# AnimatePortrait/AnimatePortrait

Measured on AMD Instinct MI355X. Metric: generator frames/sec @256x256 bs=16, higher is better.
Workload: dtype f32 (fp32 tensors; wide convs multiply fp32-class on the bf16 pipe: operands as bf16 head + tail, 3 products of 16-bit significands per multiply, ~2^-17 relative per product, fp32 accumulate); 1 GPU; Module2 generator resnet_9blocks_rcatland32_full_ifw fwd-only, ngf=64, bs=16/GPU, 256x256, fp32 (BASELINE configs[1]); global_batch=16, parallelism=dp1 (frame batches sharded, no collective), weights=random init N(0,0.02), seed 1234

## Files before the change

animateportrait_amd/csrc/conv_bf16x3.h:

```cpp
#pragma once
#include <type_traits>
#include <utility>

#include "conv_igemm.h"

namespace apamd {

typedef __bf16 bf16x8 __attribute__((ext_vector_type(8)));

template <int S_, int K_, int WCO_, int MT_, int WPX_, int NT_, int NTAP_ = 0, int ROW_ = 0, int PARTS_ = 2, int S2D3_ = 0,
          int OB16_ = 0>
struct Bf3Cfg {
    static constexpr int OB16 = OB16_;
    static_assert(!OB16_ || (K_ == 3 && S_ == 1 && PARTS_ == 1 && !ROW_), "bf16 output: the plain-bf16 3x3 stride-1 tiles");
    static constexpr int CI = 16, S = S_, K = K_, WCO = WCO_, MT = MT_, WPX = WPX_, NT = NT_, ROW = ROW_, PARTS = PARTS_;
    static constexpr int S2D3 = S2D3_;
    static_assert(!S2D3_ || (K_ == 0 && NTAP_ == 4), "compile-time s2d tap sets: the 4-tap run-time-tap family");
    static_assert(PARTS == 1 || PARTS == 2, "head only, or head + tail");
    static constexpr int TMAX = K > 0 ? (ROW ? K : K * K) : NTAP_;
    static_assert(TMAX >= 1, "K == 0 needs a tap count");
    static constexpr int EXT = K > 0 ? K - 1 : 1;
    static constexpr int EXTY = (K > 0 && ROW) ? 0 : EXT;
    static constexpr int TH = WPX * NT;
    static constexpr int CO_TILE = WCO * MT * 32;
    static constexpr int IH = (TH - 1) * S + EXTY + 1;
    static constexpr int IW = 31 * S + EXT + 1;
    static constexpr int PLANE = IH * IW;
    static constexpr int XP = (2 * PLANE + 63) / 64 * 64;
    static constexpr int X_SLOTS = PARTS * XP;
    static int w_slots(int ntaps) { return PARTS * ntaps * 2 * CO_TILE; }
    static constexpr int NIT = XP / 256 + (XP % 256 ? 1 : 0);
    static constexpr int W_BYTES_MAX = PARTS * TMAX * 2 * CO_TILE * 16;
    static constexpr int NPATCH = (NT % 2 == 0 && (8 * 32 * 36 + WPX * CO_TILE * 2) * 4 <= PARTS * XP * 16 + W_BYTES_MAX) ? 2 : 1;
    static constexpr int EPI_FLOATS = 4 * NPATCH * 32 * 36 + WPX * CO_TILE * 2;
    static_assert(WCO * WPX == 4, "4 waves per workgroup");
    static_assert(CO_TILE % 16 == 0, "weight image must be whole wave-wide LDS-DMA pieces");
    static_assert(IH < 128 && IW < 256, "piece geometry is packed into 15 bits");
    static constexpr int WG_PER_CU = (PARTS == 1 || 2 * (X_SLOTS + PARTS * TMAX * 2 * CO_TILE) * 16 + 1024 <= 80 * 1024) ? 2 : 1;
    static int wfloats(int ntaps) { return 2 * ntaps * 2 * CO_TILE * 4; }
    static size_t lds_bytes(int ntaps) {
        const size_t stage = (size_t)(X_SLOTS + w_slots(ntaps)) * 16, epi = (size_t)EPI_FLOATS * 4;
        return 2 * stage + (epi > stage ? (epi - stage + 15) / 16 * 16 : 0);
    }
};

__device__ __forceinline__ void split_bf16(float v, __bf16& hi, __bf16& lo) {
    hi = (__bf16)v;
    lo = (__bf16)(v - (float)hi);
}

struct Bf3Tile {
    int n, cot, ty, tx;
};

__device__ __forceinline__ void glds16_sv(const void* sbase, unsigned voff, unsigned lds_addr) {
    asm volatile("s_mov_b32 m0, %2\n\ts_nop 0\n\tglobal_load_lds_dwordx4 %0, %1" ::"v"(voff), "s"(sbase), "s"(lds_addr)
                 : "memory", "m0");
}
template <int IMM>
__device__ __forceinline__ void glds16_si(const void* sbase, unsigned voff, unsigned lds_base) {
    asm volatile("s_add_u32 m0, %2, %3\n\ts_nop 0\n\tglobal_load_lds_dwordx4 %0, %1" ::"v"(voff), "s"(sbase), "s"(lds_base), "n"(IMM)
                 : "memory", "m0", "scc");
}
__device__ __forceinline__ void dma_wait_all() { asm volatile("s_waitcnt vmcnt(0)" ::: "memory"); }

template <class F, int... J>
__device__ __forceinline__ void static_for_impl(F&& f, std::integer_sequence<int, J...>) {
    (f(std::integral_constant<int, J>{}), ...);
}
template <int N, class F>
__device__ __forceinline__ void static_for(F&& f) {
    static_for_impl(static_cast<F&&>(f), std::make_integer_sequence<int, N>{});
}

template <class C>
__global__ __launch_bounds__(256, C::WG_PER_CU) void conv_bf16x3(const ConvKParams p) {
    constexpr int S = C::S, K = C::K, TMAX = C::TMAX, MT = C::MT, NT = C::NT, WCO = C::WCO;
// ... 78 lines not shown
        if (p.nseg > 1 && chunk >= p.seg[1].chunk_begin) s = 1;
        if (p.nseg > 2 && chunk >= p.seg[2].chunk_begin) s = 2;
        return s;
    };

    int pgeo[NIT];
#pragma unroll
    for (int k = 0; k < NIT; ++k) {
        const int it = tid + k * 256;
        const int kg = it >= PLANE ? 1 : 0;
        const int pix = it - kg * PLANE;
        const int ly = pix / IW;
        int lx = pix - ly * IW;
        if constexpr (S == 2) lx = lx < IWE ? 2 * lx : 2 * (lx - IWE) + 1;
        pgeo[k] = it < 2 * PLANE ? ((kg << 15) | (ly << 8) | lx) : -1;
    }
    auto locate = [&](int logical, Bf3Tile& t, int (&goff)[NIT]) __attribute__((always_inline)) {
        t.cot = logical % p.co_tiles;
        int t_ = logical / p.co_tiles;
        t.tx = t_ % p.tiles_x;
        t_ /= p.tiles_x;
        t.ty = t_ % p.tiles_y;
        t.n = t_ / p.tiles_y;
        int dy0 = p.dy0, dx0 = p.dx0;
        if (p.nphase > 1) {
            const int ph = t.cot / p.co_tiles_phase;
            dy0 = p.ph_dy0[ph];
            dx0 = p.ph_dx0[ph];
        }
        const int iy0 = t.ty * C::TH * S + dy0, ix0 = t.tx * 32 * S + dx0;
#pragma unroll
        for (int k = 0; k < NIT; ++k) {
            int gy = iy0 + ((pgeo[k] >> 8) & 127), gx = ix0 + (pgeo[k] & 255);
            bool ok = pgeo[k] >= 0;
            if (p.pad_mode == 1) {
                gy = reflect_clamp(gy, H);
                gx = reflect_clamp(gx, W);
            } else {
                ok = ok && gy >= 0 && gy < H && gx >= 0 && gx < W;
            }
            goff[k] = (ok ? ((pgeo[k] >> 15) & 1) * (HW + 1) + gy * W + gx : HW) * 16;
        }
    };
    struct DmaCtx {
        const unsigned char* xh;
        const unsigned char* xl;
        const unsigned char* wsrc;
        unsigned xdst, wdst;
        unsigned wmask;
    };
    constexpr int NWP = (W_SLOTS / 64 + 3) / 4, NPIECE = PARTS * NIT + NWP;
    unsigned woff[NWP];
#pragma unroll
    for (int j = 0; j < NWP; ++j) woff[j] = ((j * 4 + wave) * 64 + lane) * 16;
    auto dma_setup = [&](int n, int cot, int chunk_, int buf) __attribute__((always_inline)) {
        const int chunk = chunk_ < nreal ? chunk_ : nreal - 1;
        const int s = seg_of(chunk);
        const int cg0 = (chunk - p.seg[s].chunk_begin) * 2;
        const int CG = p.seg[s].C >> 3;
        const unsigned char* xs = reinterpret_cast<const unsigned char*>(p.seg[s].data);
        const unsigned char* xh = xs + ((long long)(n * 2 + 0) * CG + cg0) * (HW + 1) * 16;
        const unsigned char* xl = xs + ((long long)(n * 2 + 1) * CG + cg0) * (HW + 1) * 16;
        unsigned xdst = lds0 + (buf * STAGE + W_SLOTS + wave * 64) * 16;
        const unsigned char* wsrc = reinterpret_cast<const unsigned char*>(p.wp + ((long long)cot * nchunks + chunk_) * p.wfloats);
        unsigned wdst = lds0 + (buf * STAGE + wave * 64) * 16;
        unsigned wmask = 0xFu;
        if constexpr (C::S2D3) wmask = p.s2d_mask[chunk_ / p.s2d_div < 3 ? chunk_ / p.s2d_div : 3];
        asm volatile("" : "+s"(xh), "+s"(xl), "+s"(wsrc), "+s"(xdst), "+s"(wdst));
        return DmaCtx{xh, xl, wsrc, xdst, wdst, wmask};
    };
    auto dma_piece = [&](const DmaCtx& d, const int (&goff)[NIT], const int (&alt)[NIT], bool use_alt, auto jt) __attribute__((always_inline)) {
        constexpr int j = decltype(jt)::value;
        if constexpr (j < PARTS * NIT) {
            constexpr int part = j / NIT, k = j % NIT;
            constexpr bool whole = k * 256 + 3 * 64 < XP;
            if (whole || k * 256 + wave * 64 < XP)
                glds16_si<(part * XP + k * 256) * 16>(part ? d.xl : d.xh, (unsigned)(use_alt ? alt[k] : goff[k]), d.xdst);
        } else {
            constexpr int jj = j - PARTS * NIT;
            constexpr bool whole = jj * 4 + 3 < W_SLOTS / 64;
            bool want = whole || jj * 4 + wave < W_SLOTS / 64;
            if constexpr (C::S2D3) want = want && ((d.wmask >> (((jj * 4 + wave) % (T * 2 * CO_TILE / 64)) / (2 * CO_TILE / 64))) & 1u);
            if (want) glds16_si<jj * 4096>(d.wsrc, woff[jj], d.wdst);
        }
    };
    auto issue = [&](const Bf3Tile& t, const int (&goff)[NIT], int chunk_, int buf) __attribute__((always_inline)) {
        const DmaCtx d = dma_setup(t.n, t.cot, chunk_, buf);
        static_for<NPIECE>([&](auto jt) __attribute__((always_inline)) { dma_piece(d, goff, goff, false, jt); });
    };

    const int a_slot = half * CO_TILE + wco * MT * 32 + l32;
    const int b_slot = half * PLANE + (wpx * NT) * S * IW + (S == 2 ? l32 : l32 * S);

    f32x16 acc[MT][NT];
    bf16x8 ah[2][MT], al[2][MT], bh[2][NT], bl[2][NT];
    constexpr bool WIN = (K == 4 || (K == 3 && NT > 1)) && !C::ROW && S == 1;
    constexpr int WR = WIN ? NT + K - 1 : 1;
    bf16x8 wh[2][WR], wl[2][WR];
    auto fetch_a = [&](int stage_buf, int t, int buf) __attribute__((always_inline)) {
        const uint4* Wc = wbuf + stage_buf * STAGE + a_slot;
#pragma unroll
        for (int m = 0; m < MT; ++m) {
            ah[buf][m] = *reinterpret_cast<const bf16x8*>(Wc + ((0 * T + t) * 2) * CO_TILE + m * 32);
            if constexpr (PARTS == 2) al[buf][m] = *reinterpret_cast<const bf16x8*>(Wc + ((1 * T + t) * 2) * CO_TILE + m * 32);
        }
    };
    auto fetch_brow = [&](int stage_buf, int kx, int j, int wb) __attribute__((always_inline)) {
        const uint4* Xc = xbuf + stage_buf * STAGE + b_slot + j * IW + kx;
        wh[wb][j] = *reinterpret_cast<const bf16x8*>(Xc);
        if constexpr (PARTS == 2) wl[wb][j] = *reinterpret_cast<const bf16x8*>(Xc + XP);
    };
    auto fetch = [&](int stage_buf, int t, int buf) __attribute__((always_inline)) {
        const uint4* Wc = wbuf + stage_buf * STAGE + a_slot;
        const uint4* Xc = xbuf + stage_buf * STAGE + b_slot;
        int toff;
        if constexpr (K > 0) toff = C::ROW ? t : (t / K) * IW + (S == 2 ? ((t % K) & 1) * IWE + ((t % K) >> 1) : (t % K));
        else toff = (int)((p.tap_bits >> (2 * t)) & 1u) * IW + (int)((p.tap_bits >> (2 * t + 1)) & 1u);
// ... 192 lines not shown
            }
            for (; c < 2 * cpp; c += 2) {
                stage(P0{}, std::integral_constant<unsigned, 0x5u>{}, c);
                stage(P1{}, std::integral_constant<unsigned, 0x5u>{}, c + 1);
            }
            for (; c < 3 * cpp; c += 2) {
                stage(P0{}, std::integral_constant<unsigned, 0x3u>{}, c);
                stage(P1{}, std::integral_constant<unsigned, 0x3u>{}, c + 1);
            }
            for (; c < nchunks; c += 2) {
                stage(P0{}, std::integral_constant<unsigned, 0x1u>{}, c);
                stage(P1{}, std::integral_constant<unsigned, 0x1u>{}, c + 1);
            }
        } else {
            for (int c = 0; c < nchunks; c += 2) {
                stage(P0{}, std::integral_constant<unsigned, 0u>{}, c);
                stage(P1{}, std::integral_constant<unsigned, 0u>{}, c + 1);
            }
        }
        AP_STAMP(3, 0);
        constexpr int pl = 1;

        auto epilogue = [&](auto atag) __attribute__((always_inline)) {
            constexpr int ACT = decltype(atag)::value;
            auto actf = [&](float v) { return ACT >= 0 ? apply_act(v, ACT) : apply_act(v, p.act); };
            constexpr int TS = 36;
            float* const epi = reinterpret_cast<float*>(smem + pl * STAGE);
            constexpr int NP = C::NPATCH;
            float* const patch0 = epi + wave * (NP * 32 * TS);
            float* const sred = epi + 4 * NP * 32 * TS;
            const int n = cur.n;
            int cot = cur.cot, oy_off = p.oy_off, ox_off = p.ox_off, stat_off = p.stat_tile_off;
            if (p.nphase > 1) {
                const int ph = cot / p.co_tiles_phase;
                cot -= ph * p.co_tiles_phase;
                oy_off = p.ph_oy[ph];
                ox_off = p.ph_ox[ph];
                stat_off = p.ph_stat[ph];
            }
            const int oy0 = cur.ty * C::TH, ox0 = cur.tx * 32;
            const int co_base = cot * CO_TILE + wco * MT * 32;
            const bool want_stats = p.stats != nullptr;
            const bool vec_ok = ((p.o_rstride | (int)p.o_cstride | (int)p.o_nstride) & 3) == 0 && p.osx == 1 && ox_off == 0 &&
                                (reinterpret_cast<uintptr_t>(p.y) & 15) == 0;
            const bool full = vec_ok && ox0 + 32 <= p.OW;
            const int prow = lane >> 3, pcol = (lane & 7) * 4;
            const int oxv = ox0 + pcol;
            bool octet = false;
            if constexpr (C::K == 0 || C::ROW || (C::K == 3 && C::S == 1 && C::PARTS == 2 && !C::OB16)) {
                octet = p.o_octet != 0;
                if (octet) {
                    const int ox = ox0 + l32;
                    const long long ohw = (long long)p.OH * p.OW;
                    const bool allv = !(C::WG_PER_CU == 2 && (C::K == 0 || (C::ROW && C::MT == 2))) &&
                                      __builtin_amdgcn_readfirstlane((int)(p.bias == nullptr && ACT == 0 && co_base + MT * 32 <= p.Cout &&
                                                                           oy0 + C::TH <= p.OH && ox0 + 32 <= p.OW)) != 0;
#pragma unroll
                    for (int m = 0; m < MT; ++m) {
                        float s16[16], q16[16];
#pragma unroll
                        for (int r = 0; r < 16; ++r) { s16[r] = 0.f; q16[r] = 0.f; }
                        if (allv) {
#pragma unroll
                            for (int g = 0; g < 4; ++g) {
                                const int co = co_base + m * 32 + g * 8 + 4 * half;
                                float* const ob = p.y + (long long)n * p.o_nstride + (long long)(co >> 3) * ohw * 8 + (co & 7) +
                                                  ((long long)(oy0 + wpx * NT) * p.OW + ox) * 8;
#pragma unroll
                                for (int q = 0; q < NT; ++q) {
                                    float vv[4];
#pragma unroll
                                    for (int j = 0; j < 4; ++j) {
                                        vv[j] = acc[m][q][g * 4 + j];
                                        s16[g * 4 + j] += vv[j];
                                        q16[g * 4 + j] += vv[j] * vv[j];
                                    }
                                    *reinterpret_cast<float4*>(ob + (long long)q * p.OW * 8) = make_float4(vv[0], vv[1], vv[2], vv[3]);
                                }
                            }
                        } else
#pragma unroll
                        for (int g = 0; g < 4; ++g) {
                            const int co = co_base + m * 32 + g * 8 + 4 * half;
                            const bool cok = co < p.Cout;
                            float bv[4] = {0.f, 0.f, 0.f, 0.f};
                            if (p.bias != nullptr && cok) {
#pragma unroll
                                for (int j = 0; j < 4; ++j) bv[j] = p.bias[co + j];
                            }
                            float* const obase = p.y + (long long)n * p.o_nstride + (long long)(co >> 3) * ohw * 8 + (co & 7);
#pragma unroll
                            for (int q = 0; q < NT; ++q) {
                                const int oy = oy0 + wpx * NT + q;
                                if (cok && oy < p.OH && ox < p.OW) {
                                    float vv[4];
#pragma unroll
                                    for (int j = 0; j < 4; ++j) {
                                        vv[j] = acc[m][q][g * 4 + j] + bv[j];
                                        s16[g * 4 + j] += vv[j];
                                        q16[g * 4 + j] += vv[j] * vv[j];
                                    }
                                    *reinterpret_cast<float4*>(obase + ((long long)oy * p.OW + ox) * 8) =
                                        make_float4(actf(vv[0]), actf(vv[1]), actf(vv[2]), actf(vv[3]));
                                }
                            }
                        }
                        if (want_stats) {
// ... 303 lines not shown
```

animateportrait_amd/csrc/conv_bf3_inst_taps4.hip:

```cpp
#include "conv_bf3_registry.h"
namespace apamd {
void bf3_register_taps4(std::vector<Bf3Kernel>& v) { v.push_back(bk2<1, 0, 1, 2, 4, 4, 4>("Bf3Cfg<1, 0, 1, 2, 4, 4, 4>")); }
}
```

animateportrait_amd/csrc/conv_bf3_inst_taps4_half.hip:

```cpp
#include "conv_bf3_registry.h"
namespace apamd {
void bf3_s2d3_kernels(const void*& fn, const void*& fn1);
void bf3_register_taps4_half(std::vector<Bf3Kernel>& v) {
    v.push_back(bk2<1, 0, 1, 2, 4, 2, 4>("Bf3Cfg<1, 0, 1, 2, 4, 2, 4>"));
    bf3_s2d3_kernels(v.back().fn_s2d3, v.back().fn1_s2d3);
}
}
```

animateportrait_amd/csrc/conv_bf3_registry.h:

```cpp
#pragma once
#include <vector>

#include "conv_bf16x3.h"

namespace apamd {

struct Bf3Kernel {
    int S, K, CO_TILE, TH, TMAX, ROW;
    const void* fn;
    int (*wfloats)(int);
    size_t (*lds_bytes)(int);
    const char* name;
    const void* fn1;
    size_t (*lds_bytes1)(int);
    const void* fn_s2d3 = nullptr;
    const void* fn1_s2d3 = nullptr;
    const void* fn1_ob16 = nullptr;
    const void* kernel(int precision) const { return precision == AP_PRECISION_BF16 ? fn1 : fn; }
    const void* kernel_s2d3(int precision) const { return precision == AP_PRECISION_BF16 ? fn1_s2d3 : fn_s2d3; }
    size_t lds(int precision, int ntaps) const { return precision == AP_PRECISION_BF16 ? lds_bytes1(ntaps) : lds_bytes(ntaps); }
};

template <int S, int K, int WCO, int MT, int WPX, int NT, int NTAP = 0, int ROW = 0>
static Bf3Kernel bk2(const char* name) {
    using C = Bf3Cfg<S, K, WCO, MT, WPX, NT, NTAP, ROW, 2>;
    using C1 = Bf3Cfg<S, K, WCO, MT, WPX, NT, NTAP, ROW, 1>;
    return Bf3Kernel{C::S, C::K, C::CO_TILE, C::TH, C::TMAX, C::ROW, reinterpret_cast<const void*>(&conv_bf16x3<C>),
                     &C::wfloats, &C::lds_bytes, name, reinterpret_cast<const void*>(&conv_bf16x3<C1>), &C1::lds_bytes};
}

void bf3_register_k3_tall(std::vector<Bf3Kernel>&);
void bf3_register_k3_short(std::vector<Bf3Kernel>&);
void bf3_register_s2k3(std::vector<Bf3Kernel>&);
void bf3_register_k4(std::vector<Bf3Kernel>&);
void bf3_register_row_tall(std::vector<Bf3Kernel>&);
void bf3_register_row_half(std::vector<Bf3Kernel>&);
void bf3_register_taps12(std::vector<Bf3Kernel>&);
void bf3_register_taps4(std::vector<Bf3Kernel>&);
void bf3_register_taps4_half(std::vector<Bf3Kernel>&);
const Bf3Kernel* ph4_kernel(int KK);

}
```

animateportrait_amd/csrc/conv_host.hip:

```cpp
#include "common.h"
#include "conv_registry.h"
#include "conv_direct.h"
#include "conv_bf3_registry.h"
#include "conv_prepass.h"
#include "conv_small.h"
#include "conv_head.h"
#include "conv_tsmall.h"

#include <cstdlib>
#include <cstring>
#include <vector>

namespace apamd {

#ifdef APAMD_VARIANTS
const void* bf3_sb_kernel(size_t* lds_bytes);
#endif

static thread_local char g_err[512];
char* last_error_buf() { return g_err; }
int fail(int code, const char* fmt, ...) {
    va_list ap;
    va_start(ap, fmt);
    vsnprintf(g_err, sizeof(g_err), fmt, ap);
    va_end(ap);
    return code;
}

static const std::vector<ConvKernelInfo>& registry() {
    static std::vector<ConvKernelInfo> v;
    static std::once_flag once;
    std::call_once(once, [] {
        register_s1k0(v);
        register_s1k3(v);
        register_s1k4(v);
        register_s1k7(v);
        register_s2k3(v);
        register_s2k4(v);
    });
    return v;
}

static const ConvKernelInfo* find_kernel(int CI, int S, int K, int CO_TILE) {
    for (const auto& k : registry())
        if (k.CI == CI && k.S == S && k.K == K && k.CO_TILE == CO_TILE) return &k;
    return nullptr;
}

static const std::vector<Bf3Kernel>& bf3_registry() {
    static std::vector<Bf3Kernel> v;
    static std::once_flag once;
    std::call_once(once, [] {
        bf3_register_k3_short(v);
        bf3_register_k3_tall(v);
        bf3_register_s2k3(v);
        bf3_register_k4(v);
        bf3_register_row_tall(v);
        bf3_register_row_half(v);
        bf3_register_taps12(v);
        bf3_register_taps4(v);
        bf3_register_taps4_half(v);
    });
    return v;
}
static const Bf3Kernel* bf3_for_taps(const Bf3Kernel* k, int ntaps) {
    if (k->K != 0) return k;
    for (const auto& e : bf3_registry())
        if (e.K == 0 && e.S == k->S && e.TMAX == ntaps && e.TH == k->TH) return &e;
    return nullptr;
}

struct Tap { int ky, kx, ly, lx; };

struct Launch {
    std::vector<Tap> taps;
    int OH, OW, dy0, dx0;
    int osy, osx, oy_off, ox_off;
    int tiles_x, tiles_y;
    long long wp_off;
    int stat_tile_off;
};

struct Plan {
    const ConvKernelInfo* k = nullptr;
    int direct_cop = 0;
    bool small = false;
    bool head = false;
    bool tsmall = false;
    long long head_w_off = -1;
    bool bf3 = false;
    bool fused_phases = false;
    int ph4 = 0;
    bool k0_small = false;
    const Bf3Kernel* bk = nullptr;
    std::vector<Launch> launches;
    int Cin = 0, nchunks = 0, cin_pad = 0, co_tiles = 0;
    int chunk_begin[kMaxSeg] = {0, 0, 0};
    int Hout = 0, Wout = 0, stat_tiles = 0;
    long long packed_floats = 0;
};

struct Geom {
    bool rowk;
    int K;
    int S, KT;
};

static int plan_geometry(const ap_conv_desc* d, Plan& pl, Geom& g) {
    if (!d) return fail(AP_ERR_INVALID, "null descriptor");
    if (d->nsrc < 1 || d->nsrc > kMaxSeg) return fail(AP_ERR_INVALID, "nsrc=%d out of range", d->nsrc);
    if (d->N < 1 || d->H < 1 || d->W < 1 || d->Cout < 1) return fail(AP_ERR_INVALID, "bad dims");
    g.rowk = d->KH == 1 && d->KW == 7;
    if (g.rowk) {
        if (d->transposed || d->stride != 1 || d->pad != 3 || d->nsrc != 1 || d->src[0].C != 32 ||
            d->precision == AP_PRECISION_FP32 || d->w_layout != AP_W_OIHW || d->w_flip)
            return fail(AP_ERR_UNSUPPORTED, "1x7 kernels exist only as the row form of a 7x7 stem (one 32-channel "
                                            "split source, stride 1, pad 3, split-bf16 precision)");
        if (d->pad_mode == AP_PAD_REFLECT && d->pad >= d->W) return fail(AP_ERR_INVALID, "reflection pad %d >= width", d->pad);
    } else if (d->KH != d->KW || d->KH < 1 || d->KH > 7) {
        return fail(AP_ERR_UNSUPPORTED, "kernel %dx%d", d->KH, d->KW);
    }
    const int K = g.K = d->KW;
    if (g.rowk) {
        g.S = 1; g.KT = K;
        pl.Hout = d->H; pl.Wout = d->W;
    } else if (!d->transposed) {
        if (d->stride != 1 && d->stride != 2) return fail(AP_ERR_UNSUPPORTED, "stride %d", d->stride);
        g.S = d->stride; g.KT = K;
        if (K == 2) {
            if (d->stride != 1 || d->pad != 0 || d->precision == AP_PRECISION_FP32 || d->w_layout != AP_W_OIHW || d->w_flip)
                return fail(AP_ERR_UNSUPPORTED, "2x2 kernels exist only as the space-to-depth form of a 4x4 stride-2 layer "
                                                "(stride 1, pad 0, split-bf16 precision)");
            g.KT = 0;
        } else if (K == 1) {
            if (d->stride != 1 || d->pad != 0) return fail(AP_ERR_UNSUPPORTED, "1x1 kernels: stride 1, pad 0 only");
            g.KT = 0;
        } else if (K != 3 && K != 4 && K != 7) {
            return fail(AP_ERR_UNSUPPORTED, "kernel size %d (built: 1, 3, 4, 7)", K);
        }
        pl.Hout = (d->H + 2 * d->pad - K) / g.S + 1;
        pl.Wout = (d->W + 2 * d->pad - K) / g.S + 1;
        if (d->pad_mode == AP_PAD_REFLECT && (d->pad >= d->H || d->pad >= d->W))
            return fail(AP_ERR_INVALID, "reflection pad %d >= input size", d->pad);
    } else {
        if (d->stride != 2) return fail(AP_ERR_UNSUPPORTED, "transposed conv needs stride 2");
        if (d->pad_mode != AP_PAD_ZERO) return fail(AP_ERR_UNSUPPORTED, "transposed conv with reflection pad");
        g.S = 1; g.KT = 0;
        pl.Hout = (d->H - 1) * 2 - 2 * d->pad + K + d->output_padding;
        pl.Wout = (d->W - 1) * 2 - 2 * d->pad + K + d->output_padding;
    }
    if (pl.Hout < 1 || pl.Wout < 1) return fail(AP_ERR_INVALID, "empty output");
    pl.Cin = 0;
    for (int s = 0; s < d->nsrc; ++s) {
        if (d->src[s].C < 1) return fail(AP_ERR_INVALID, "segment %d has C=%d", s, d->src[s].C);
        pl.Cin += d->src[s].C;
    }
    return AP_OK;
}

static void layout_chunks(const ap_conv_desc* d, Plan& pl, int ci) {
    pl.nchunks = 0;
    for (int s = 0; s < d->nsrc; ++s) {
        pl.chunk_begin[s] = pl.nchunks;
        pl.nchunks += (d->src[s].C + ci - 1) / ci;
    }
    pl.cin_pad = pl.nchunks * ci;
}

static bool plan_direct(const ap_conv_desc* d, const Geom& g, Plan& pl) {
    if (g.rowk || d->transposed || d->stride != 1 || g.K != 7 || d->pad != 3 || d->Cout > 4) return false;
    pl.direct_cop = d->Cout == 1 ? 1 : 4;
    layout_chunks(d, pl, 4);
    pl.packed_floats = (long long)pl.cin_pad * g.K * g.K * pl.direct_cop;
    pl.stat_tiles = ((pl.Hout + 15) / 16) * ((pl.Wout + 63) / 64);
    return true;
}

static bool plan_small(const ap_conv_desc* d, const Geom& g, Plan& pl) {
    if (g.rowk || d->transposed || g.K != 3 || d->nsrc != 1 || pl.Cin > 16 || (d->Cout != 8 && d->Cout != 16) ||
        d->w_layout != AP_W_OIHW || d->w_flip || env_int("APAMD_NO_SMALL", 0))
        return false;
    pl.small = true;
    pl.nchunks = 1;
    pl.cin_pad = pl.Cin;
    pl.packed_floats = (long long)d->Cout * pl.Cin * 9;
    pl.stat_tiles = ((pl.Hout + 7) / 8) * ((pl.Wout + 31) / 32);
    return true;
}

static bool plan_head_tsmall(const ap_conv_desc* d, const Geom& g, Plan& pl) {
    const bool head_w = !g.rowk && !d->transposed && d->stride == 1 && g.K == 4 && d->Cout == 1 && d->nsrc == 1 && pl.Cin >= 64 &&
                        d->w_layout == AP_W_OIHW && !d->w_flip && d->pad == 1;
    pl.head = head_w && d->W <= kHeadMaxW;
    pl.tsmall = !g.rowk && d->transposed && d->stride == 2 && g.K == 4 && d->pad == 1 && d->output_padding == 0 && d->Cout <= 4 &&
                d->nsrc == 1 && d->w_layout == AP_W_IOHW && !d->w_flip;
    return head_w || pl.tsmall;
}

static int pick_bf3(const ap_conv_desc* d, const Geom& g, Plan& pl) {
    const int K = g.K, KT = g.KT;
    if (g.rowk) {
        for (const auto& k : bf3_registry())
            if (k.ROW && k.K == K && (!pl.bk || k.TH < pl.bk->TH)) pl.bk = &k;
        return pl.bk ? AP_OK : fail(AP_ERR_UNSUPPORTED, "no 1x%d row kernel", K);
    }
    if (d->precision == AP_PRECISION_FP32 || !(d->Cout >= 48 || (d->Cout >= 16 && pl.Cin >= 128)) || pl.Cin < 32 ||
        env_int("APAMD_NO_BF16X3", 0))
        return AP_OK;
    for (int s = 0; s < d->nsrc; ++s)
        if (d->src[s].C % 16 != 0) return AP_OK;
    if (!(KT == 0 ? K <= 4 : (K == 3 || (K == 4 && g.S == 1)))) return AP_OK;
    const Bf3Kernel *tall = nullptr, *small = nullptr;
    for (const auto& k : bf3_registry())
        if (k.S == g.S && k.K == KT && !k.ROW) {
            if (!tall || k.TH >= tall->TH) tall = &k;
            if (!small || k.TH < small->TH) small = &k;
        }
    pl.bk = tall;
    const bool even_out = pl.Hout % 2 == 0 && pl.Wout % 2 == 0;
    if (KT == 0) {
        pl.k0_small = K == 2 || K == 4 || (d->transposed && K == 3 && even_out);
        if (pl.k0_small) pl.bk = small;
        if (d->transposed && (K == 3 || K == 4) && d->pad == 1 && d->stride == 2 && even_out) {
            pl.ph4 = K;
            pl.bk = ph4_kernel(K);
        }
    } else if (tall && small != tall) {
        const long long tiles = (long long)d->N * ((pl.Hout + tall->TH - 1) / tall->TH) * ((pl.Wout + 31) / 32) *
                                ((d->Cout + tall->CO_TILE - 1) / tall->CO_TILE);
        if ((tiles * 2 <= num_cus() || pl.Hout <= small->TH) && !env_int("APAMD_NO_SMALL_TILES", 0)) pl.bk = small;
    }
    return AP_OK;
}

static int pick_igemm(const ap_conv_desc* d, const Geom& g, Plan& pl) {
    int co_tile = d->Cout >= 96 ? 128 : (d->Cout >= 48 ? 64 : 32);
    co_tile = env_int("APAMD_CONV_COTILE", co_tile);
    int minC = 1 << 30;
    for (int s = 0; s < d->nsrc; ++s) minC = std::min(minC, (int)d->src[s].C);
    int ci = minC <= 2 ? 2 : (minC <= 4 ? 4 : 8);
    for (int s = 0; s < d->nsrc; ++s)
        while (ci > 2 && d->src[s].C % ci != 0 && d->src[s].C > ci) ci >>= 1;
    const int ntaps_max = d->transposed ? ((g.K + 1) / 2) * ((g.K + 1) / 2) : g.K * g.K;
    const size_t lds_target = (size_t)env_int("APAMD_CONV_LDS_TARGET", 72 * 1024);
    for (;;) {
        const ConvKernelInfo* k = find_kernel(ci, g.S, g.KT, co_tile);
        if (!k) return fail(AP_ERR_UNSUPPORTED, "no kernel for CI=%d S=%d K=%d CO_TILE=%d", ci, g.S, g.KT, co_tile);
        int nch = 0;
        for (int s = 0; s < d->nsrc; ++s) nch += (d->src[s].C + ci - 1) / ci;
        const size_t bytes = 4 * k->lds_floats(ntaps_max, nch > 1 ? 2 : 1, nch * ci);
        if (bytes <= lds_target || ci == 2) {
            if (bytes > 160 * 1024) return fail(AP_ERR_UNSUPPORTED, "LDS tile of %zu bytes does not fit", bytes);
            pl.k = k;
            break;
        }
        ci >>= 1;
    }
    if (const int forced = env_int("APAMD_CONV_CI", 0)) {
        if (const ConvKernelInfo* k = find_kernel(forced, g.S, g.KT, co_tile)) { pl.k = k; ci = forced; }
    }
    layout_chunks(d, pl, ci);
    pl.co_tiles = (d->Cout + co_tile - 1) / co_tile;
    return AP_OK;
}

static void add_launch(Plan& pl, Launch& L) {
    const int ntaps = (int)L.taps.size();
    const int th = pl.bk ? pl.bk->TH : pl.k->TH;
    const int wf = pl.bk ? pl.bk->wfloats(ntaps) : pl.k->wfloats(ntaps);
    L.tiles_x = (L.OW + 31) / 32;
    L.tiles_y = (L.OH + th - 1) / th;
    L.wp_off = pl.packed_floats;
    L.stat_tile_off = pl.stat_tiles;
    pl.packed_floats += (long long)pl.co_tiles * pl.nchunks * wf;
    pl.stat_tiles += L.tiles_x * L.tiles_y;
// ... 301 lines not shown
    if (!src || !src->data || !out) return fail(AP_ERR_INVALID, "split_prepass_rows: null pointer");
    if (K != 7 || pad != 3 || src->C < 1 || src->C > 4)
        return fail(AP_ERR_UNSUPPORTED, "split_prepass_rows: built for 7x7 stems with 1..4 input channels (K=%d, C=%d)", K, src->C);
    if (N < 1 || N > 65535 || H < 1 || W < 1) return fail(AP_ERR_INVALID, "split_prepass_rows: bad sizes");
    if ((src->mean == nullptr) != (src->rstd == nullptr)) return fail(AP_ERR_INVALID, "split_prepass_rows: mean/rstd mismatch");
    if (pad_mode == AP_PAD_REFLECT && pad >= H) return fail(AP_ERR_INVALID, "split_prepass_rows: reflection pad %d >= height", pad);
    SplitRowsParams p;
    memset(&p, 0, sizeof(p));
    p.x = src->data; p.mean = src->mean; p.rstd = src->rstd; p.act = src->act;
    p.N = N; p.C = src->C; p.H = H; p.W = W; p.K = K; p.pad = pad; p.pad_mode = pad_mode;
    p.out = reinterpret_cast<uint4*>(out);
    const dim3 grid((H * W + 255) / 256, N);
    switch (src->C) {
        case 1: hipLaunchKernelGGL((split_rows_kernel<7, 1>), grid, dim3(256), 0, (hipStream_t)stream, p); break;
        case 2: hipLaunchKernelGGL((split_rows_kernel<7, 2>), grid, dim3(256), 0, (hipStream_t)stream, p); break;
        case 3: hipLaunchKernelGGL((split_rows_kernel<7, 3>), grid, dim3(256), 0, (hipStream_t)stream, p); break;
        default: hipLaunchKernelGGL((split_rows_kernel<7, 4>), grid, dim3(256), 0, (hipStream_t)stream, p); break;
    }
    return check_launch("split_rows_kernel");
}

int ap_split_prepass_s2d(const ap_src* src, int32_t N, int32_t H, int32_t W, void* out, ap_stream_t stream) {
    if (!src || !src->data || !out) return fail(AP_ERR_INVALID, "split_prepass_s2d: null pointer");
    if (src->C < 8 || src->C % 8 != 0 || H < 2 || W < 2 || (H & 1) || (W & 1))
        return fail(AP_ERR_UNSUPPORTED, "split_prepass_s2d: needs channels in multiples of 8 and an even map (C=%d, %dx%d)",
                    src->C, H, W);
    if (N < 1 || N > 65535 || src->C / 2 > 65535) return fail(AP_ERR_INVALID, "split_prepass_s2d: bad sizes");
    if ((src->mean == nullptr) != (src->rstd == nullptr)) return fail(AP_ERR_INVALID, "split_prepass_s2d: mean/rstd mismatch");
    if (src->act < 0 || src->act > 2) return fail(AP_ERR_INVALID, "split_prepass_s2d: act %d", src->act);
    SplitS2dParams p;
    memset(&p, 0, sizeof(p));
    p.x = src->data; p.mean = src->mean; p.rstd = src->rstd; p.act = src->act;
    p.N = N; p.C = src->C; p.H = H; p.W = W;
    p.out = reinterpret_cast<uint4*>(out);
    const int HW2 = (H / 2 + 1) * (W / 2 + 1);
    hipLaunchKernelGGL(split_s2d_kernel, dim3((HW2 + 255) / 256, src->C / 2, N), dim3(256), 0, (hipStream_t)stream, p);
    return check_launch("split_s2d_kernel");
}

int ap_split_prepass(const ap_src* src, int32_t N, int32_t H, int32_t W, void* out, ap_stream_t stream) {
    if (!src || !out) return fail(AP_ERR_INVALID, "split_prepass: null pointer");
    return ap_norm_apply_split(src, nullptr, 0, 0.f, nullptr, nullptr, nullptr, N, H, W, nullptr, out, stream);
}

int ap_conv2d_kernel_name(const ap_conv_desc* d, char* buf, int32_t buflen) {
    Plan pl;
    int rc = make_plan(d, pl);
    if (rc) return rc;
    if (!buf || buflen < 1) return fail(AP_ERR_INVALID, "kernel_name: bad buffer");
    if (pl.direct_cop) snprintf(buf, buflen, "DirectCfg<%d, %d>", d->KH, pl.direct_cop);
    else if (pl.small) snprintf(buf, buflen, "SmallCfg<%d, %d>", d->stride, d->Cout);
    else if (pl.head) snprintf(buf, buflen, "HeadCfg<%d>", d->KH);
    else if (pl.tsmall) snprintf(buf, buflen, "TSmallCfg<%d>", d->Cout);
    else if (pl.bf3) snprintf(buf, buflen, "%s%s", pl.bk->name, d->precision == AP_PRECISION_BF16 ? " bf16" : "");
    else snprintf(buf, buflen, "ConvCfg<%d, %d, %d, %d, %d, %d, %d>", pl.k->CI, pl.k->S, pl.k->K, pl.k->WCO, pl.k->MT, pl.k->WPX, pl.k->NT);
    return AP_OK;
}

int ap_conv2d_pack_weights(const ap_conv_desc* d, const float* weight, float* packed, ap_stream_t stream) {
    Plan pl;
    int rc = make_plan(d, pl);
    if (rc) return rc;
    if (!weight || !packed) return fail(AP_ERR_INVALID, "null weight/packed pointer");
    if (pl.small) {
        hipError_t e = hipMemcpyAsync(packed, weight, (size_t)pl.packed_floats * sizeof(float), hipMemcpyDeviceToDevice,
                                      (hipStream_t)stream);
        if (e != hipSuccess) return fail(AP_ERR_LAUNCH, "pack (copy) weights: %s", hipGetErrorString(e));
        return AP_OK;
    }
    if (pl.direct_cop) {
        PackDirectParams p;
        memset(&p, 0, sizeof(p));
        p.w = weight; p.out = packed;
        p.Cin = pl.Cin; p.Cout = d->Cout; p.K = d->KH; p.layout = d->w_layout; p.flip = d->w_flip;
        p.COP = pl.direct_cop; p.CI = 4; p.nchunks = pl.nchunks; p.nseg = d->nsrc;
        for (int s = 0; s < d->nsrc; ++s) { p.segC[s] = d->src[s].C; p.chunk_begin[s] = pl.chunk_begin[s]; }
        hipLaunchKernelGGL(pack_direct_kernel, dim3(64), dim3(256), 0, (hipStream_t)stream, p);
        return check_launch("pack_direct_kernel");
    }
    if (pl.bf3) {
        for (const auto& L : pl.launches) {
            const PackBf3Params p = bf3_pack_params(d, pl, L, weight, nullptr, packed);
            hipLaunchKernelGGL(pack_bf16x3_kernel, dim3(1024), dim3(256), 0, (hipStream_t)stream, p);
            rc = check_launch("pack_bf16x3_kernel");
            if (rc) return rc;
        }
        return AP_OK;
    }
    for (const auto& L : pl.launches) {
        PackParams p;
        memset(&p, 0, sizeof(p));
        p.w = weight;
        p.out = packed + L.wp_off;
        p.Cin = pl.Cin; p.Cout = d->Cout; p.K = d->KH; p.layout = d->w_layout;
        p.nseg = d->nsrc;
        for (int s = 0; s < d->nsrc; ++s) { p.segC[s] = d->src[s].C; p.chunk_begin[s] = pl.chunk_begin[s]; }
        p.CI = pl.k->CI; p.CO_TILE = pl.k->CO_TILE; p.nchunks = pl.nchunks; p.co_tiles = pl.co_tiles;
        p.ntaps = (int)L.taps.size();
        p.wfloats = pl.k->wfloats(p.ntaps);
        for (int t = 0; t < p.ntaps; ++t) { p.tap_ky[t] = L.taps[t].ky; p.tap_kx[t] = L.taps[t].kx; }
        const long long total = (long long)p.co_tiles * p.nchunks * p.wfloats;
        int blocks = (int)std::min<long long>((total + 255) / 256, 2048);
        hipLaunchKernelGGL(pack_weights_kernel, dim3(blocks), dim3(256), 0, (hipStream_t)stream, p);
        rc = check_launch("pack_weights_kernel");
        if (rc) return rc;
    }
    if (pl.head_w_off >= 0) {
// ... 243 lines not shown
        p.ph_dy0[ph] = Lp.dy0; p.ph_dx0[ph] = Lp.dx0; p.ph_oy[ph] = Lp.oy_off; p.ph_ox[ph] = Lp.ox_off;
        p.ph_stat[ph] = Lp.stat_tile_off;
        p.ph_tapmask[ph] = phase_tapmask(Lp);
    }
}

static void s2d3_params(ConvKParams& p, const ap_conv_desc* d, const Plan& pl) {
    if (d->s2d_k != 3 || d->transposed || pl.bk->K != 0 || d->KW != 2 || d->nsrc != 1 || d->src[0].C % 64 != 0) return;
    p.s2d_div = d->src[0].C / 64;
    for (int r = 0; r < 4; ++r) {
        p.s2d_mask[r] = 0;
        for (int t = 0; t < 4; ++t)
            if (2 * (t >> 1) + (r >> 1) <= 2 && 2 * (t & 1) + (r & 1) <= 2) p.s2d_mask[r] |= 1u << t;
    }
}

static unsigned bf3_workgroups(long long tiles, size_t lds, bool two_per_cu) {
    int cus = num_cus() * ((2 * lds <= 160 * 1024 || two_per_cu) ? 2 : 1);
    if (const int forced = env_int("APAMD_BF3_BLOCKS", 0)) {
        static bool told = false;
        if (!told) fprintf(stderr, "libapamd: APAMD_BF3_BLOCKS=%d overrides the persistent workgroup count\n", forced);
        told = true;
        cus = forced;
    }
    return (unsigned)(tiles > cus ? cus : tiles);
}

static int launch_bf3(const ap_conv_desc* d, const Plan& pl, const OutForm& o, const FwdArgs& a) {
    if (!d->presplit)
        return fail(AP_ERR_INVALID, "this layer runs on the split-bf16 path: pass sources prepared by "
                                    "ap_split_prepass and set desc.presplit (see ap_conv2d_wants_presplit)");
    int rc = pl.ph4 ? check_ph4_plan(pl, o.view) : AP_OK;
    if (rc) return rc;
    for (const auto& L : pl.launches) {
        const Bf3Kernel* kern = pl.ph4 ? pl.bk : bf3_for_taps(pl.bk, (int)L.taps.size());
        if (!kern) return fail(AP_ERR_UNSUPPORTED, "no split-bf16 kernel for a phase with %d taps", (int)L.taps.size());
        ConvKParams p = conv_params(d, pl, L, a, false);
        p.wfloats = pl.bk->wfloats(p.ntaps);
        p.o_octet = o.octet ? 1 : 0;
        if (const ap_out_view* v = o.view) {
            p.OH = v->OH; p.OW = v->OW;
            p.tiles_x = (v->OW + 31) / 32;
            p.tiles_y = (v->OH + pl.bk->TH - 1) / pl.bk->TH;
            p.o_nstride = v->nstride; p.o_cstride = v->cstride; p.o_rstride = v->rstride;
            p.osy = 1; p.oy_off = v->y_off;
            p.osx = v->xstride; p.ox_off = v->x_off * v->xstride;
        }
        if (pl.fused_phases) fused_phase_params(p, pl);
        s2d3_params(p, d, pl);
        if (pl.bk->K == 0 && (rc = tap_bits(L, p.tap_bits))) return rc;
        const void* kfn = o.bf16 ? kern->fn1_ob16 : kern->kernel(d->precision);
        if (p.s2d_div > 0 && (p.s2d_div & 1) == 0 && p.nchunks == 4 * p.s2d_div && kern->kernel_s2d3(d->precision))
            kfn = kern->kernel_s2d3(d->precision);
        rc = ensure_dyn_lds(kfn, 160 * 1024);
        if (rc) return rc;
        size_t lds = kern->lds(d->precision, p.ntaps);
        bool sb = false;
#ifdef APAMD_VARIANTS
        if (!o.view && !o.octet && kern->K == 3 && kern->S == 1 && kern->TH == 16 && !kern->ROW && d->precision != AP_PRECISION_BF16 &&
            p.osx == 1 && p.osy == 1 && p.oy_off == 0 && p.ox_off == 0 && env_int("APAMD_CONV_SB", 0)) {
            kfn = bf3_sb_kernel(&lds);
            rc = ensure_dyn_lds(kfn, 160 * 1024);
            if (rc) return rc;
            p.sb_skew = env_int("APAMD_CONV_SB_SKEW", 0);
            sb = true;
        }
#endif
#ifdef APAMD_ABLATION
        if (const char* sb_ = getenv("APAMD_STAMP_BUF")) {
            const int words = env_int("APAMD_STAMP_WORDS", 512);
            if (!pl.ph4 && lds + (size_t)16 * words <= 160 * 1024) {
                p.stamps = reinterpret_cast<unsigned*>(strtoull(sb_, nullptr, 0));
                p.stamp_lds_off = (int)lds;
                p.stamp_words = words;
                lds += (size_t)16 * words;
            }
        }
#endif
        if (lds > 160 * 1024) return fail(AP_ERR_UNSUPPORTED, "bf16x3 LDS tile of %zu bytes does not fit", lds);
        if (p.nchunks < 2) return fail(AP_ERR_UNSUPPORTED, "bf16x3 pipeline needs >= 32 input channels");
        if (((long long)d->H * d->W + 1) * 32 >= (1LL << 31))
            return fail(AP_ERR_UNSUPPORTED, "split-bf16 path: %d x %d planes are too large", d->H, d->W);
        const unsigned nblk = bf3_workgroups((long long)d->N * p.tiles_y * p.tiles_x * p.co_tiles, lds, sb);
        void* args[] = {&p};
        hipError_t e = hipLaunchKernel(kfn, dim3(nblk), dim3(256), args, lds, a.stream);
        if (e != hipSuccess) return fail(AP_ERR_LAUNCH, "conv_bf16x3 launch: %s", hipGetErrorString(e));
        if (pl.fused_phases) break;
    }
    return AP_OK;
}

static int conv2d_fwd_impl(const ap_conv_desc* d, const OutForm& o, const FwdArgs& a) {
    Plan pl;
    int rc = make_plan(d, pl);
    if (rc) return rc;
    rc = check_fwd_args(d, pl, o, a);
    if (rc) return rc;
    if (pl.tsmall && !a.stats) return launch_tsmall(d, pl, a);
    if (pl.head && !a.stats) return launch_head(d, pl, a);
    if (pl.small) return launch_small(d, pl, a);
    if (pl.bf3) return launch_bf3(d, pl, o, a);
    if (pl.direct_cop) return launch_direct(d, pl, a);
    return launch_igemm(d, pl, a);
}

}

extern "C" {

// ... 41 lines not shown
```

animateportrait_amd/csrc/conv_igemm.h:

```cpp
#pragma once
#include <hip/hip_runtime.h>
#include <stdint.h>
#include "common.h"

namespace apamd {

typedef float f32x16 __attribute__((ext_vector_type(16)));

constexpr int kMaxTaps = 49;
constexpr int kMaxSeg = 3;

struct SrcSeg {
    const float* data;
    const float* mean;
    const float* rstd;
    int C;
    int act;
    int chunk_begin;
    int pad_;
};

struct ConvKParams {
    SrcSeg seg[kMaxSeg];
    int nseg;
    int N, H, W;
    int Cout;
    int OH, OW;
    int dy0, dx0;
    int pad_mode;
    float* y;
    long long o_nstride;
    long long o_cstride;
    int o_rstride;
    int osy, osx, oy_off, ox_off;
    const float* wp;
    const float* bias;
    int act;
    float* stats;
    int stat_tiles;
    int stat_tile_off;
    int ntaps;
    int nchunks;
    int tiles_x, tiles_y, co_tiles;
    int cin_pad;
    int wfloats;
    int ablate;
    unsigned tap_bits;
    int nphase, co_tiles_phase;
    int ph_dy0[4], ph_dx0[4], ph_oy[4], ph_ox[4], ph_stat[4];
    int s2d_div;
    unsigned s2d_mask[4];
    unsigned ph_tapmask[4];
    int o_octet;
    unsigned* stamps;
    int stamp_lds_off, stamp_words;
    int sb_skew;
};

template <int CI_, int S_, int K_, int WCO_, int MT_, int WPX_, int NT_>
struct ConvCfg {
    static constexpr int CI = CI_, S = S_, K = K_, WCO = WCO_, MT = MT_, WPX = WPX_, NT = NT_;
    static constexpr int EXT = K_ > 0 ? K_ - 1 : 1;
    static constexpr int TH = WPX * NT;
    static constexpr int CO_TILE = WCO * MT * 32;
    static constexpr int IH = (TH - 1) * S + EXT + 1;
    static constexpr int IW = 31 * S + EXT + 1;
    static constexpr int PLANE = IH * IW;
    static constexpr int XE = CI * PLANE;
    static constexpr int NE = (XE + 255) / 256;
    static constexpr int MINW = (MT * NT <= 4 && NE <= 6) ? 3 : (NE <= 24 ? 2 : 1);
    static_assert(WCO * WPX == 4, "4 waves per workgroup");
    static_assert(CI % 2 == 0, "channel chunk must hold whole (ci, ci+1) pairs");
    static int wfloats(int ntaps) { return (ntaps * CI * CO_TILE + 255) / 256 * 256; }
    static size_t lds_floats(int ntaps, int nbuf, int cin_pad) {
        size_t f = (size_t)nbuf * ((size_t)wfloats(ntaps) + XE) + 2 * (size_t)cin_pad;
        size_t red = (size_t)WPX * CO_TILE * 2;
        return f > red ? f : red;
    }
};

__device__ __forceinline__ int reflect_clamp(int i, int n) {
    i = i < 0 ? -i : i;
    i = i >= n ? 2 * (n - 1) - i : i;
    i = i < 0 ? 0 : (i >= n ? n - 1 : i);
    return i;
}

__device__ __forceinline__ void glds16(const float* gsrc, float* ldst) {
    __builtin_amdgcn_global_load_lds((const __attribute__((address_space(1))) void*)gsrc,
                                     (__attribute__((address_space(3))) void*)ldst, 16, 0, 0);
}

__device__ __forceinline__ float apply_act(float v, int act) {
    if (act == 1) return v > 0.f ? v : 0.f;
    if (act == 2) return v > 0.f ? v : 0.2f * v;
    if (act == 3) return tanhf(v);
    return v;
}

template <class C>
__global__ __launch_bounds__(256, C::MINW) void conv_igemm_f32(const ConvKParams p) {
    constexpr int CI = C::CI, S = C::S, MT = C::MT, NT = C::NT, WCO = C::WCO;
    constexpr int IW = C::IW, PLANE = C::PLANE, XE = C::XE, NE = C::NE, CO_TILE = C::CO_TILE;
    extern __shared__ __attribute__((aligned(16))) float smem[];

// ... 293 lines not shown
```

Baseline: 2285 frames/s.

## Add wide and tall tile variants for space-to-depth 3x3 bf16x3 convs

Adds two new kernel instantiations for space-to-depth 3x3 (4-tap) convolutions: a tall 16-row tile and a wide 128-cout x 8-row tile. The wide tile stitches two packed 64-cout weight blocks per workgroup, with odd and even waves loading separate halves. A heuristic picks the wide tile when Cout > 64 and there are enough tiles to fill the CUs; an env var can force short, tall or wide. The goal is more input reuse per staged activation tile, at the cost of one workgroup per CU and the octet all-valid fast path being disabled for these tiles.

```diff
diff --git a/animateportrait_amd/csrc/conv_bf16x3.h b/animateportrait_amd/csrc/conv_bf16x3.h
--- a/animateportrait_amd/csrc/conv_bf16x3.h
+++ b/animateportrait_amd/csrc/conv_bf16x3.h
@@ -23,6 +23,8 @@
     static constexpr int EXTY = (K > 0 && ROW) ? 0 : EXT;
     static constexpr int TH = WPX * NT;
     static constexpr int CO_TILE = WCO * MT * 32;
+    static constexpr int WHALF = (S2D3_ && CO_TILE == 128) ? 1 : 0;
+    static_assert(!S2D3_ || CO_TILE == 64 || CO_TILE == 128, "space-to-depth 3x3 tiles: one or two packed 64-cout blocks");
     static constexpr int IH = (TH - 1) * S + EXTY + 1;
     static constexpr int IW = 31 * S + EXT + 1;
     static constexpr int PLANE = IH * IW;
@@ -207,7 +209,7 @@
     constexpr int NWP = (W_SLOTS / 64 + 3) / 4, NPIECE = PARTS * NIT + NWP;
     unsigned woff[NWP];
 #pragma unroll
-    for (int j = 0; j < NWP; ++j) woff[j] = ((j * 4 + wave) * 64 + lane) * 16;
+    for (int j = 0; j < NWP; ++j) woff[j] = (((j * 4 + wave) >> C::WHALF) * 64 + lane) * 16;
     auto dma_setup = [&](int n, int cot, int chunk_, int buf) __attribute__((always_inline)) {
         const int chunk = chunk_ < nreal ? chunk_ : nreal - 1;
         const int s = seg_of(chunk);
@@ -217,7 +219,12 @@
         const unsigned char* xh = xs + ((long long)(n * 2 + 0) * CG + cg0) * (HW + 1) * 16;
         const unsigned char* xl = xs + ((long long)(n * 2 + 1) * CG + cg0) * (HW + 1) * 16;
         unsigned xdst = lds0 + (buf * STAGE + W_SLOTS + wave * 64) * 16;
-        const unsigned char* wsrc = reinterpret_cast<const unsigned char*>(p.wp + ((long long)cot * nchunks + chunk_) * p.wfloats);
+        int wblk = cot;
+        if constexpr (C::WHALF) {
+            wblk = 2 * cot + (wave & 1);
+            if (wblk >= p.w_tiles64) wblk = p.w_tiles64 - 1;
+        }
+        const unsigned char* wsrc = reinterpret_cast<const unsigned char*>(p.wp + ((long long)wblk * nchunks + chunk_) * p.wfloats);
         unsigned wdst = lds0 + (buf * STAGE + wave * 64) * 16;
         unsigned wmask = 0xFu;
         if constexpr (C::S2D3) wmask = p.s2d_mask[chunk_ / p.s2d_div < 3 ? chunk_ / p.s2d_div : 3];
@@ -516,7 +523,7 @@
                 if (octet) {
                     const int ox = ox0 + l32;
                     const long long ohw = (long long)p.OH * p.OW;
-                    const bool allv = !(C::WG_PER_CU == 2 && (C::K == 0 || (C::ROW && C::MT == 2))) &&
+                    const bool allv = !C::S2D3 && !(C::WG_PER_CU == 2 && (C::K == 0 || (C::ROW && C::MT == 2))) &&
                                       __builtin_amdgcn_readfirstlane((int)(p.bias == nullptr && ACT == 0 && co_base + MT * 32 <= p.Cout &&
                                                                            oy0 + C::TH <= p.OH && ox0 + 32 <= p.OW)) != 0;
 #pragma unroll
diff --git a/animateportrait_amd/csrc/conv_bf3_inst_s2d3_tall.hip b/animateportrait_amd/csrc/conv_bf3_inst_s2d3_tall.hip
--- /dev/null
+++ b/animateportrait_amd/csrc/conv_bf3_inst_s2d3_tall.hip
@@ -0,0 +1,4 @@
+#include "conv_bf3_registry.h"
+namespace apamd {
+const void* bf3_s2d3_tall_kernel() { return reinterpret_cast<const void*>(&conv_bf16x3<Bf3Cfg<1, 0, 1, 2, 4, 4, 4, 0, 2, 1>>); }
+}
diff --git a/animateportrait_amd/csrc/conv_bf3_inst_s2d3_wide.hip b/animateportrait_amd/csrc/conv_bf3_inst_s2d3_wide.hip
--- /dev/null
+++ b/animateportrait_amd/csrc/conv_bf3_inst_s2d3_wide.hip
@@ -0,0 +1,9 @@
+#include "conv_bf3_registry.h"
+namespace apamd {
+void bf3_s2d3_wide_kernel(const void*& fn, size_t (*&lds_bytes)(int)) {
+    using C = Bf3Cfg<1, 0, 2, 2, 2, 4, 4, 0, 2, 1>;
+    static_assert(C::CO_TILE == 128 && C::TH == 8 && C::WG_PER_CU == 1, "128 couts x 8 rows, one workgroup per CU");
+    fn = reinterpret_cast<const void*>(&conv_bf16x3<C>);
+    lds_bytes = &C::lds_bytes;
+}
+}
diff --git a/animateportrait_amd/csrc/conv_bf3_inst_taps4.hip b/animateportrait_amd/csrc/conv_bf3_inst_taps4.hip
--- a/animateportrait_amd/csrc/conv_bf3_inst_taps4.hip
+++ b/animateportrait_amd/csrc/conv_bf3_inst_taps4.hip
@@ -1,4 +1,8 @@
 #include "conv_bf3_registry.h"
 namespace apamd {
-void bf3_register_taps4(std::vector<Bf3Kernel>& v) { v.push_back(bk2<1, 0, 1, 2, 4, 4, 4>("Bf3Cfg<1, 0, 1, 2, 4, 4, 4>")); }
+const void* bf3_s2d3_tall_kernel();
+void bf3_register_taps4(std::vector<Bf3Kernel>& v) {
+    v.push_back(bk2<1, 0, 1, 2, 4, 4, 4>("Bf3Cfg<1, 0, 1, 2, 4, 4, 4>"));
+    v.back().fn_s2d3 = bf3_s2d3_tall_kernel();
 }
+}
diff --git a/animateportrait_amd/csrc/conv_bf3_inst_taps4_half.hip b/animateportrait_amd/csrc/conv_bf3_inst_taps4_half.hip
--- a/animateportrait_amd/csrc/conv_bf3_inst_taps4_half.hip
+++ b/animateportrait_amd/csrc/conv_bf3_inst_taps4_half.hip
@@ -1,8 +1,11 @@
 #include "conv_bf3_registry.h"
 namespace apamd {
 void bf3_s2d3_kernels(const void*& fn, const void*& fn1);
+void bf3_s2d3_wide_kernel(const void*& fn, size_t (*&lds_bytes)(int));
 void bf3_register_taps4_half(std::vector<Bf3Kernel>& v) {
     v.push_back(bk2<1, 0, 1, 2, 4, 2, 4>("Bf3Cfg<1, 0, 1, 2, 4, 2, 4>"));
     bf3_s2d3_kernels(v.back().fn_s2d3, v.back().fn1_s2d3);
+    bf3_s2d3_wide_kernel(v.back().fn_s2d3_wide, v.back().lds_bytes_s2d3_wide);
+    v.back().name_s2d3_wide = "Bf3Cfg<1, 0, 2, 2, 2, 4, 4>";
 }
 }
diff --git a/animateportrait_amd/csrc/conv_bf3_registry.h b/animateportrait_amd/csrc/conv_bf3_registry.h
--- a/animateportrait_amd/csrc/conv_bf3_registry.h
+++ b/animateportrait_amd/csrc/conv_bf3_registry.h
@@ -15,6 +15,9 @@
     size_t (*lds_bytes1)(int);
     const void* fn_s2d3 = nullptr;
     const void* fn1_s2d3 = nullptr;
+    const void* fn_s2d3_wide = nullptr;
+    size_t (*lds_bytes_s2d3_wide)(int) = nullptr;
+    const char* name_s2d3_wide = nullptr;
     const void* fn1_ob16 = nullptr;
     const void* kernel(int precision) const { return precision == AP_PRECISION_BF16 ? fn1 : fn; }
     const void* kernel_s2d3(int precision) const { return precision == AP_PRECISION_BF16 ? fn1_s2d3 : fn_s2d3; }
diff --git a/animateportrait_amd/csrc/conv_host.hip b/animateportrait_amd/csrc/conv_host.hip
--- a/animateportrait_amd/csrc/conv_host.hip
+++ b/animateportrait_amd/csrc/conv_host.hip
@@ -70,6 +70,8 @@
     return nullptr;
 }
 
+enum { kS2d3Short = 0, kS2d3Tall = 1, kS2d3Wide = 2 };
+
 struct Tap { int ky, kx, ly, lx; };
 
 struct Launch {
@@ -92,6 +94,7 @@
     bool fused_phases = false;
     int ph4 = 0;
     bool k0_small = false;
+    int s2d3_tile = kS2d3Short;
     const Bf3Kernel* bk = nullptr;
     std::vector<Launch> launches;
     int Cin = 0, nchunks = 0, cin_pad = 0, co_tiles = 0;
@@ -197,6 +200,22 @@
     return head_w || pl.tsmall;
 }
 
+static bool s2d3_layer(const ap_conv_desc* d) {
+    return d->s2d_k == 3 && !d->transposed && d->KW == 2 && d->nsrc == 1 && d->src[0].C % 128 == 0;
+}
+
+static int choose_s2d3_tile(const ap_conv_desc* d, const Plan& pl) {
+    if (!s2d3_layer(d) || d->precision != AP_PRECISION_BF16X3) return kS2d3Short;
+    const bool tall_ok = pl.Hout > 8, wide_ok = d->Cout > 64;
+    if (const char* f = getenv("APAMD_S2D3_TILE")) {
+        if (!strcmp(f, "short")) return kS2d3Short;
+        if (!strcmp(f, "tall")) return tall_ok ? kS2d3Tall : kS2d3Short;
+        if (!strcmp(f, "wide")) return wide_ok ? kS2d3Wide : kS2d3Short;
+    }
+    const long long wide_tiles = (long long)d->N * ((pl.Hout + 7) / 8) * ((pl.Wout + 31) / 32) * ((d->Cout + 127) / 128);
+    return wide_ok && wide_tiles >= num_cus() ? kS2d3Wide : kS2d3Short;
+}
+
 static int pick_bf3(const ap_conv_desc* d, const Geom& g, Plan& pl) {
     const int K = g.K, KT = g.KT;
     if (g.rowk) {
@@ -221,6 +240,9 @@
     if (KT == 0) {
         pl.k0_small = K == 2 || K == 4 || (d->transposed && K == 3 && even_out);
         if (pl.k0_small) pl.bk = small;
+        pl.s2d3_tile = K == 2 ? choose_s2d3_tile(d, pl) : kS2d3Short;
+        if (pl.s2d3_tile == kS2d3Tall && tall->kernel_s2d3(d->precision)) pl.bk = tall;
+        else if (pl.s2d3_tile != kS2d3Wide || !small->fn_s2d3_wide) pl.s2d3_tile = kS2d3Short;
         if (d->transposed && (K == 3 || K == 4) && d->pad == 1 && d->stride == 2 && even_out) {
             pl.ph4 = K;
             pl.bk = ph4_kernel(K);
@@ -628,7 +650,8 @@
     else if (pl.small) snprintf(buf, buflen, "SmallCfg<%d, %d>", d->stride, d->Cout);
     else if (pl.head) snprintf(buf, buflen, "HeadCfg<%d>", d->KH);
     else if (pl.tsmall) snprintf(buf, buflen, "TSmallCfg<%d>", d->Cout);
-    else if (pl.bf3) snprintf(buf, buflen, "%s%s", pl.bk->name, d->precision == AP_PRECISION_BF16 ? " bf16" : "");
+    else if (pl.bf3) snprintf(buf, buflen, "%s%s", pl.s2d3_tile == kS2d3Wide ? pl.bk->name_s2d3_wide : pl.bk->name,
+                              d->precision == AP_PRECISION_BF16 ? " bf16" : "");
     else snprintf(buf, buflen, "ConvCfg<%d, %d, %d, %d, %d, %d, %d>", pl.k->CI, pl.k->S, pl.k->K, pl.k->WCO, pl.k->MT, pl.k->WPX, pl.k->NT);
     return AP_OK;
 }
@@ -978,9 +1001,15 @@
         const void* kfn = o.bf16 ? kern->fn1_ob16 : kern->kernel(d->precision);
         if (p.s2d_div > 0 && (p.s2d_div & 1) == 0 && p.nchunks == 4 * p.s2d_div && kern->kernel_s2d3(d->precision))
             kfn = kern->kernel_s2d3(d->precision);
+        size_t lds = kern->lds(d->precision, p.ntaps);
+        if (pl.s2d3_tile == kS2d3Wide) {
+            kfn = kern->fn_s2d3_wide;
+            lds = kern->lds_bytes_s2d3_wide(p.ntaps);
+            p.w_tiles64 = pl.co_tiles;
+            p.co_tiles = (d->Cout + 127) / 128;
+        }
         rc = ensure_dyn_lds(kfn, 160 * 1024);
         if (rc) return rc;
-        size_t lds = kern->lds(d->precision, p.ntaps);
         bool sb = false;
 #ifdef APAMD_VARIANTS
         if (!o.view && !o.octet && kern->K == 3 && kern->S == 1 && kern->TH == 16 && !kern->ROW && d->precision != AP_PRECISION_BF16 &&
diff --git a/animateportrait_amd/csrc/conv_igemm.h b/animateportrait_amd/csrc/conv_igemm.h
--- a/animateportrait_amd/csrc/conv_igemm.h
+++ b/animateportrait_amd/csrc/conv_igemm.h
@@ -51,6 +51,7 @@
     int s2d_div;
     unsigned s2d_mask[4];
     unsigned ph_tapmask[4];
+    int w_tiles64;
     int o_octet;
     unsigned* stamps;
     int stamp_lds_off, stamp_words;
```

New measurement: 2286 frames/s (median of 2 runs). About the same (+0.0%).
